# yondonfu/ai-rtc-agent

Hardware: NVIDIA H100
Metric: frames/sec at 512x512 SD-Turbo img2img (1-step, stream-batch 1) (higher is better)
Workload: dtype f16

## Files before the change

ai-rtc-agent_b200/csrc/engine.cu:

```cuda
#include <cuda_fp16.h>
#include <cuda_runtime.h>
#include <math.h>
#include <stddef.h>
#include <stdio.h>
#include <stdlib.h>
#include <string.h>

#include <algorithm>
#include <atomic>
#include <chrono>
#include <functional>
#include <thread>
#include <map>
#include <memory>
#include <string>
#include <vector>

#include "../../include/b200sd.h"
#include "attention.cuh"
#include "elementwise.cuh"
#include "igemm.cuh"
#include "tconv.cuh"

using namespace b2;

namespace b2 {
void igemm_record(const IgemmDesc& g, const IgemmPlan* plan, b2sd_igemm_desc* d, b2sd_igemm_plan_info* info);
}

#define CUDA_OK(expr)                                                                       \
    do {                                                                                    \
        cudaError_t e__ = (expr);                                                           \
        if (e__ != cudaSuccess) {                                                           \
            b2_set_error("%s failed: %s (%s:%d)", #expr, cudaGetErrorString(e__), __FILE__, __LINE__); \
            return -1;                                                                      \
        }                                                                                   \
    } while (0)
#define TRY(expr)            \
    do {                     \
        if ((expr) != 0) return -1; \
    } while (0)

namespace {

struct Act {
    __half* p = nullptr;
    int n = 0, h = 0, w = 0, c = 0, ld = 0;
    long elems() const { return (long)n * h * w * ld; }
};

struct Raw {
    __half* p = nullptr;
    bool pack_only = false;
    bool derived = false;
    std::vector<int64_t> shape;
    std::vector<float> host;
    long numel() const {
        long v = 1;
        for (auto s : shape) v *= s;
        return v;
    }
};

class Arena {
  public:
    explicit Arena(size_t slab) : slab_(slab) {}
    ~Arena() { release(); }
    void set_order(cudaStream_t order, cudaMemPool_t pool) { order_ = order; pool_ = pool; }
    void* alloc(size_t bytes) {
        bytes = (bytes + 1023) & ~size_t(1023);
        if (cur_ < 0 || off_ + bytes > sizes_[cur_]) {
            int next = cur_ + 1;
            while (next < (int)slabs_.size() && sizes_[next] < bytes) ++next;
            if (next >= (int)slabs_.size()) {
                size_t sz = bytes > slab_ ? bytes : slab_;
                void* p = nullptr;
                cudaError_t e = order_ ? cudaMallocFromPoolAsync(&p, sz, pool_, order_) : cudaMalloc(&p, sz);
                if (e == cudaSuccess && order_) e = cudaStreamSynchronize(order_);
                if (e != cudaSuccess) {
                    b2_set_error("device allocation of %zu bytes failed: %s", sz, cudaGetErrorString(e));
                    return nullptr;
                }
                slabs_.push_back(p);
                sizes_.push_back(sz);
                next = (int)slabs_.size() - 1;
            }
            cur_ = next;
            off_ = 0;
        }
        void* r = static_cast<char*>(slabs_[cur_]) + off_;
        off_ += bytes;
        return r;
    }
    void reset() { cur_ = slabs_.empty() ? -1 : 0; off_ = 0; }
    void release() {
        for (void* p : slabs_) order_ ? cudaFreeAsync(p, order_) : cudaFree(p);
        slabs_.clear();
        sizes_.clear();
        cur_ = -1;
        off_ = 0;
    }

  private:
    size_t slab_;
    cudaStream_t order_ = nullptr;
    cudaMemPool_t pool_ = nullptr;
    std::vector<void*> slabs_;
    std::vector<size_t> sizes_;
    int cur_ = -1;
    size_t off_ = 0;
};

struct Op {
    std::function<int(cudaStream_t)> fn;
    std::string name;
    double flops = 0.0;
    b2sd_launch_record rec{};
    template <class F>
    Op(F f, std::string n = "", double fl = 0.0) : fn(std::move(f)), name(std::move(n)), flops(fl) {}
    template <class F>
    Op(F f, std::string n, const b2sd_launch_record& r) : fn(std::move(f)), name(std::move(n)), rec(r) {}
    int operator()(cudaStream_t s) const { return fn(s); }
};

b2sd_launch_record smallconv_record(const SmallConvArgs& a) {
    b2sd_launch_record r{};
    r.kind = B2SD_LAUNCH_SMALLCONV;
    r.smallconv = b2sd_smallconv_args{a.x, a.wt, a.bias, a.y, a.ldy, a.nb, a.h, a.w_, a.cin, a.cout, a.in_h, a.in_w, a.flags,
                                      a.res, a.ldr, (int64_t)a.res_bstride, a.in_off};
    return r;
}
b2sd_launch_record upsample2x_record(const void* x, void* y, int nb, int h, int w, int c) {
    b2sd_launch_record r{};
    r.kind = B2SD_LAUNCH_UPSAMPLE2X;
    r.upsample2x = b2sd_upsample2x_args{x, y, nb, h, w, c};
    return r;
}
b2sd_launch_record post_u8_record(const void* y, int ldy, void* out, int nb, int h, int w) {
    b2sd_launch_record r{};
    r.kind = B2SD_LAUNCH_POST_U8;
    r.post_u8 = b2sd_post_u8_args{y, ldy, out, nb, h, w};
    return r;
}
b2sd_launch_record small_linear_record(const float* in, int in_ld, const void* w, const float* bias, float* out, int out_ld,
                                       int nb, int n, int k, int silu_in) {
    b2sd_launch_record r{};
    r.kind = B2SD_LAUNCH_SMALL_LINEAR;
    r.small_linear = b2sd_small_linear_args{in, in_ld, w, bias, out, out_ld, nb, n, k, silu_in};
    return r;
}

}

static int igemm_autotile_single(IgemmDesc d, bool allow_swap, IgemmPlan* plan_out);

int igemm_autotile(IgemmDesc d, bool allow_swap, IgemmPlan* plan_out) {
    TRY(igemm_autotile_single(d, allow_swap, plan_out));
    static const char* pair_env = getenv("B2_PAIR");
    static const char* ps_env = getenv("B2_PAIR_SPLITS");
    static const bool pair_single = getenv("B2_PAIR_SINGLE") != nullptr;
    const int pair_mode = pair_env ? atoi(pair_env) : d.pair_auto;
    const int pair_splits = ps_env ? atoi(ps_env) : (d.pair_splits > 0 ? d.pair_splits : 4);
    const IgemmPlan& pl = *plan_out;
    const int m_tiles = pl.p.tiles_w * pl.p.tiles_h * pl.p.tiles_n;
    if (pair_mode <= 0 || pl.p.swap || m_tiles < 2 || (pl.p.BN % 32) != 0 || (d.epi.flags & (IG_SILU | IG_PAD0))) return 0;
    if (pair_mode == 2 && pl.p.total_kb < 20) return 0;
    d.swap = 0; d.BN = pl.p.BN; d.splits = pl.splits > pair_splits ? pair_splits : pl.splits; d.partial = nullptr;
    d.pair = pair_single ? 0 : 1;
    IgemmPlan paired;
    if (igemm_plan(d, &paired)) return 0;
    *plan_out = paired;
    return 0;
}

static int igemm_autotile_single(IgemmDesc d, bool allow_swap, IgemmPlan* plan_out) {
    IgemmPlan& plan = *plan_out;
    const bool geglu = (d.epi.flags & IG_GEGLU) != 0;
    const bool silu = (d.epi.flags & IG_SILU) != 0;
    const bool pad0 = (d.epi.flags & IG_PAD0) != 0;
    const int n_gemm = geglu ? 2 * d.epi.n_valid : d.epi.n_valid;
    static const bool swap_on = getenv("B2_SWAP") != nullptr, swap_off = getenv("B2_NO_SWAP") != nullptr;
    static const bool tuned = getenv("B2_NO_TUNED_TILES") == nullptr;
    static const char* ms_env = getenv("B2_MAX_SPLITS");
    const int max_splits = ms_env ? atoi(ms_env) : (d.max_splits > 0 ? d.max_splits : 8);
    int total_kb = 0;
    for (int sidx = 0; sidx < d.nseg && sidx < IG_MAX_SRC; ++sidx) total_kb += d.ntap[sidx] * (d.src[sidx].C / IG_BK);
    const long rows_all = (long)d.Nb * d.Ho * d.Wo;
    const bool swap_here = allow_swap && !geglu && !pad0 && d.epi.n_valid >= 128 && (d.epi.n_valid & 7) == 0 &&
                           (swap_on || (!swap_off && tuned && rows_all <= 64 && total_kb >= 90));
    if (swap_here) {
        d.swap = 1;
        d.BN = rows_all >= 256 ? 256 : (rows_all >= 128 ? 128 : 64);
        d.splits = 1; d.partial = nullptr;
        TRY(igemm_plan(d, &plan));
        const long ctas = (long)plan.grid.x * plan.grid.y;
        int max_by_k = plan.p.total_kb / 4;
        if (max_by_k < 1) max_by_k = 1;
        if (max_by_k > 8) max_by_k = 8;
        int splits = 1;
        while (splits * 2 <= max_by_k && ctas * splits * 2 <= 192 && splits * 2 <= max_splits) splits *= 2;
        if (splits > 1) {
            d.splits = splits;
            TRY(igemm_plan(d, &plan));
        }
        return 0;
    }
    d.swap = 0;
    auto vt_ok = [&](int bn) { return !d.epi.out2 || d.epi.col2 % bn == 0; };
    if (tuned && !geglu && !silu && !pad0 && n_gemm % 160 == 0 && total_kb >= 40 && vt_ok(160)) {
        d.BN = 160; d.splits = 1; d.partial = nullptr;
        TRY(igemm_plan(d, &plan));
        const int m_tiles = plan.p.tiles_w * plan.p.tiles_h * plan.p.tiles_n;
        const long tiles = (long)m_tiles * (n_gemm / 160);
        int bn = 0, splits = 0;
        if (tiles < 132) {
            if (m_tiles >= 8) { bn = 160; splits = 4; }
            else if (m_tiles >= 2 && n_gemm % 256 == 0 && total_kb >= 180 && vt_ok(256)) { bn = 256; splits = 8; }
        }
        if (bn && splits > max_splits) bn = 0;
        if (bn) {
            d.BN = bn; d.splits = splits;
            TRY(igemm_plan(d, &plan));
            return 0;
        }
    }
    static const int cands[] = {256, 160, 128, 64, 32, 16};
    std::vector<int> valid;
    for (int bn : cands) {
        if (geglu && (bn % 32 != 0 || bn < 64)) continue;
        if (silu && (bn > 128 || bn % 16 || (bn & (bn - 1)))) continue;
        if (pad0 && bn != 64 && bn != 128 && bn != 256) continue;
        if (n_gemm % bn == 0 && vt_ok(bn)) valid.push_back(bn);
    }
    if (valid.empty()) {
        int bn = 16;
        while (bn < n_gemm && bn < 128) bn <<= 1;
        valid.push_back(bn);
    }
    for (int bn : valid) {
        if (bn < 64 && n_gemm >= 64) break;
        d.BN = bn; d.splits = 1; d.partial = nullptr;
        TRY(igemm_plan(d, &plan));
        if (plan.p.acc_bufs == 2 || (long)plan.grid.x * plan.grid.y >= b2_device_sms()) return 0;
    }
    int bn = valid.back();
    for (int v : valid) if (v >= 64) bn = v;
    d.BN = bn; d.splits = 1; d.partial = nullptr;
    TRY(igemm_plan(d, &plan));
    const long ctas = (long)plan.grid.x * plan.grid.y;
    int splits = ctas >= 96 ? 1 : (int)((IG_SMS + ctas - 1) / ctas);
    if (tuned && ctas >= 64 && total_kb <= 12) splits = 1;
    const int max_by_k = plan.p.total_kb / 4 > 0 ? plan.p.total_kb / 4 : 1;
    if (splits > max_by_k) splits = max_by_k;
    if (splits > 8) splits = 8;
    while (splits > max_splits && splits > 1) splits >>= 1;
    if (geglu) splits = 1;
    if (splits > 1) {
        d.splits = splits;
        TRY(igemm_plan(d, &plan));
    }
    return 0;
}

struct WeightStore {
    std::shared_ptr<WeightStore> parent;
    struct OrderStream {
        cudaStream_t s = nullptr;
        cudaMemPool_t pool = nullptr;
        ~OrderStream() {
            if (s) cudaStreamDestroy(s);
            if (pool) cudaMemPoolDestroy(pool);
        }
    } order;
    const uint64_t id = next_id();
    uint64_t family = id;
    struct Copy { __half* dst; const __half* src; size_t bytes; };
    std::vector<Copy> pending;
    static uint64_t next_id() {
        static std::atomic<uint64_t> n{1};
        return n++;
    }

    std::map<std::string, Raw> raw;
    Arena weights{256u << 20};
    Arena raw_only{256u << 20};
    bool raw_released = false;
    bool imported = false;
    std::map<std::string, __half*> packed;
    std::map<std::string, float*> fvec;
    std::map<std::string, size_t> packed_bytes, fvec_bytes;
    std::shared_ptr<struct CondPool> cond_pool;

    struct Rebuild {
        std::vector<std::string> keys;
        std::function<int(cudaStream_t)> fn;
    };
    std::map<std::string, Rebuild> rebuild;
    std::map<std::string, const __half*> src_override;
    const __half* src(const std::string& key) const {
        auto o = src_override.find(key);
        if (o != src_override.end()) return o->second;
        auto it = raw.find(key);
        return it == raw.end() ? nullptr : it->second.p;
    }
    bool live = false;
    bool live_ready = false;
    Arena base_arena{256u << 20};
    std::map<std::string, __half*> base;
    std::vector<std::string> fused;
    void* scratch = nullptr;
    size_t scratch_cap = 0;
    ~WeightStore() {
        if (scratch) order.s ? cudaFreeAsync(scratch, order.s) : cudaFree(scratch);
    }
};

enum { COND_PROMPT = 0, COND_TIME = 1 };
static const uint64_t COND_GLOBAL = 0, COND_UNKNOWN = ~0ull;

struct CondPool {
    cudaMemPool_t pool = nullptr;
    cudaStream_t reaper = nullptr;
    ~CondPool() {
// ... 39 lines not shown
    std::map<std::string, Raw>& raw;
    Arena& weights;
    Arena& raw_only;
    bool& raw_released;
    bool& imported;
    std::map<std::string, __half*>& packed;
    std::map<std::string, float*>& fvec;
    std::map<std::string, size_t>& packed_bytes;
    std::map<std::string, size_t>& fvec_bytes;
    Arena state{16u << 20};
    Arena prog{512u << 20};
    explicit b2sd_engine(std::shared_ptr<WeightStore> s)
        : ws(std::move(s)), raw(ws->raw), weights(ws->weights), raw_only(ws->raw_only), raw_released(ws->raw_released),
          imported(ws->imported), packed(ws->packed), fvec(ws->fvec), packed_bytes(ws->packed_bytes), fvec_bytes(ws->fvec_bytes) {}

    Act x_in;
    __half* noise = nullptr;
    float* coef = nullptr;
    float* tsteps = nullptr;
    __half* ctx = nullptr;
    float* temb_sin = nullptr;
    float* temb_h = nullptr;
    float* temb = nullptr;
    float* cn_temb_h = nullptr;
    float* cn_temb = nullptr;
    float* gn_ws = nullptr;
    int* tile_counters = nullptr;
    float coef_host[4][64]{};

    __half* ctx_global = nullptr;
    float* tsteps_global = nullptr;

    struct CondBlock {
        char* p = nullptr;
        char* global = nullptr;
        size_t cap = 0, used = 0;
        uint64_t held = 0;
        void* take(size_t bytes) {
            bytes = (bytes + 1023) & ~size_t(1023);
            if (used + bytes > cap) {
                b2_set_error("conditioning block of %zu bytes exhausted", cap);
                return nullptr;
            }
            void* r = p + used;
            used += bytes;
            return r;
        }
    } cond[2];
    int64_t cond_binds = 0;

    unsigned long long* ln_stats = nullptr;
    size_t ln_stats_cap = 0, ln_stats_used = 0;
    std::vector<Op> prog_frame, prog_prompt, prog_time;
    std::map<std::string, Act> taps;
    SmallConvArgs head{};
    SmallConvArgs cn_head{};
    SmallConvArgs hed_head{};
    Act image;
    bool built = false;
    int concurrency = 1;
    int launches = 0;
    std::string cur;
    bool allow_swap = false;
    size_t idx_enc_end = 0, idx_unet_end = 0;
    enum { GRAPH_WHOLE = 0, GRAPH_STAGE = 1, NUM_GRAPHS = 4 };
    cudaGraphExec_t graph_exec[NUM_GRAPHS] = {};
    void drop_graphs() {
        for (auto& g : graph_exec)
            if (g) { cudaGraphExecDestroy(g); g = nullptr; }
    }

    ~b2sd_engine() { drop_graphs(); }

    const Raw* get(const std::string& key) {
        auto it = raw.find(key);
        if (it == raw.end()) {
            b2_set_error("missing weight '%s'", key.c_str());
            return nullptr;
        }
        return &it->second;
    }
    bool has(const std::string& key) const { return raw.count(key) != 0; }

    float* vec(const std::vector<std::string>& keys, const std::vector<int>* perm = nullptr, int pad_to = 0) {
        std::string ck = "v:";
        for (auto& k : keys) ck += k + "+";
        if (perm) ck += "perm";
        auto it = fvec.find(ck);
        if (it != fvec.end()) return it->second;
        std::vector<float> host;
        for (auto& k : keys) {
            const Raw* r = get(k);
            if (!r) return nullptr;
            if (host.empty()) host.assign(r->host.begin(), r->host.end());
            else
                for (size_t i = 0; i < host.size() && i < r->host.size(); ++i) host[i] += r->host[i];
        }
        if (perm) {
            std::vector<float> t(perm->size());
            for (size_t i = 0; i < perm->size(); ++i) t[i] = (*perm)[i] >= 0 ? host[(*perm)[i]] : 0.f;
            host.swap(t);
        }
        if ((int)host.size() < pad_to) host.resize(pad_to, 0.f);
        float* d = static_cast<float*>(weights.alloc(host.size() * sizeof(float)));
        if (!d) return nullptr;
        if (cudaMemcpy(d, host.data(), host.size() * sizeof(float), cudaMemcpyHostToDevice) != cudaSuccess) return nullptr;
        fvec[ck] = d;
        fvec_bytes[ck] = host.size() * sizeof(float);
        return d;
    }

    const Raw* pack_source(const std::string& key) {
        const Raw* r = get(key);
        if (r && !r->p) {
            b2_set_error("parameter '%s' was released after the first prepare and is not in the packed cache", key.c_str());
            return nullptr;
        }
        return r;
    }
    int record_rebuild(const std::string& name, std::vector<std::string> keys, std::function<int(cudaStream_t)> fn, cudaStream_t s) {
        WeightStore::Rebuild& rb = ws->rebuild[name];
        rb.keys = std::move(keys);
        rb.fn = std::move(fn);
        return rb.fn(s);
    }

    const float* small_w(const std::string& key, cudaStream_t s) {
        auto it = fvec.find("sw:" + key);
        if (it != fvec.end()) return it->second;
        const Raw* r = pack_source(key);
        if (!r) return nullptr;
        const int cout = (int)r->shape[0], cin = (int)r->shape[1];
        float* d = static_cast<float*>(weights.alloc((size_t)cin * 9 * cout * sizeof(float)));
        WeightStore* w = ws.get();
        if (!d || record_rebuild("sw:" + key, {key}, [=](cudaStream_t st) { return smallconv_prep_launch(w->src(key), d, cout, cin, st); }, s))
            return nullptr;
        fvec["sw:" + key] = d;
        fvec_bytes["sw:" + key] = (size_t)cin * 9 * cout * sizeof(float);
        return d;
    }

    struct ConvSeg { std::string key; int c0, cn, taps; };
    __half* pack_conv(const std::string& name, const std::vector<ConvSeg>& segs, int rows, int* k_out,
                      cudaStream_t s) {
        int K = 0;
        for (auto& g : segs) K += g.taps * g.cn;
        *k_out = K;
        auto it = packed.find(name);
        if (it != packed.end()) return it->second;
        const int rows_pad = (rows + 15) / 16 * 16;
        __half* dst = static_cast<__half*>(weights.alloc((size_t)rows_pad * K * 2));
        if (!dst) return nullptr;
        std::vector<std::string> keys;
        std::vector<int> cin_total;
        for (auto& g : segs) {
            const Raw* r = pack_source(g.key);
            if (!r) return nullptr;
            keys.push_back(g.key);
            cin_total.push_back((int)r->shape[1]);
        }
        WeightStore* w = ws.get();
        const size_t bytes = (size_t)rows_pad * K * 2;
        if (record_rebuild(name, keys, [=](cudaStream_t st) {
                if (cudaMemsetAsync(dst, 0, bytes, st) != cudaSuccess) return -1;
                int koff = 0;
                for (size_t i = 0; i < segs.size(); ++i) {
                    const ConvSeg& g = segs[i];
                    if (pack_conv_weight_launch(w->src(g.key), dst, K, koff, rows, cin_total[i], g.taps, g.c0, g.cn, st)) return -1;
                    koff += g.taps * g.cn;
                }
                return 0;
            }, s))
            return nullptr;
        packed[name] = dst;
        packed_bytes[name] = bytes;
        return dst;
    }
    std::function<int(cudaStream_t)> gather_fn(const std::vector<std::pair<std::string, std::vector<int>>>& parts, int K,
                                               __half* dst, size_t bytes, cudaStream_t s) {
        std::vector<std::pair<std::string, const int*>> dparts;
        std::vector<int> counts;
        for (auto& p : parts) {
            if (!pack_source(p.first)) return nullptr;
            int* dperm = static_cast<int*>(weights.alloc(p.second.size() * sizeof(int)));
            if (!dperm) return nullptr;
            cudaMemcpyAsync(dperm, p.second.data(), p.second.size() * sizeof(int), cudaMemcpyHostToDevice, s);
            cudaStreamSynchronize(s);
            dparts.emplace_back(p.first, dperm);
            counts.push_back((int)p.second.size());
        }
        WeightStore* w = ws.get();
        return [=](cudaStream_t st) {
            if (cudaMemsetAsync(dst, 0, bytes, st) != cudaSuccess) return -1;
            size_t r0 = 0;
            for (size_t i = 0; i < dparts.size(); ++i) {
                if (gather_rows_launch(w->src(dparts[i].first), K, dparts[i].second, dst + r0 * K, K, counts[i], K, st)) return -1;
                r0 += counts[i];
            }
            return 0;
        };
    }
    static std::vector<std::string> part_keys(const std::vector<std::pair<std::string, std::vector<int>>>& parts) {
        std::vector<std::string> k;
        for (auto& p : parts) k.push_back(p.first);
        return k;
    }
    __half* pack_rows(const std::string& name, const std::vector<std::pair<std::string, std::vector<int>>>& parts,
                      int K, cudaStream_t s) {
        auto it = packed.find(name);
        if (it != packed.end()) return it->second;
        size_t rows = 0;
        for (auto& p : parts) rows += p.second.size();
        const size_t rows_pad = (rows + 15) / 16 * 16;
        __half* dst = static_cast<__half*>(weights.alloc(rows_pad * K * 2));
        if (!dst) return nullptr;
        auto gather = gather_fn(parts, K, dst, rows_pad * K * 2, s);
        if (!gather || record_rebuild(name, part_keys(parts), gather, s)) return nullptr;
        packed[name] = dst;
        packed_bytes[name] = rows_pad * K * 2;
        return dst;
    }

    struct LnFold { __half* w = nullptr; const float* colsum = nullptr; const float* bias = nullptr; };
    int fold_ln(const std::string& name, const std::vector<std::pair<std::string, std::vector<int>>>& parts, int K,
                const std::string& ln_prefix, const float* bias_vec, LnFold* out, cudaStream_t s) {
        size_t rows = 0;
        for (auto& p : parts) rows += p.second.size();
        const size_t rows_pad = (rows + 15) / 16 * 16;
        const bool done = packed.count(name) && fvec.count(name + ":cs") && fvec.count(name + ":b");
        if (!done) {
            __half* w = static_cast<__half*>(weights.alloc(rows_pad * K * 2));
            if (!w) return -1;
            auto gather = gather_fn(parts, K, w, rows_pad * K * 2, s);
            const float* gamma = vec({ln_prefix + ".weight"});
            const float* beta = vec({ln_prefix + ".bias"});
            float* cs = static_cast<float*>(weights.alloc(rows_pad * sizeof(float)));
            float* bb = static_cast<float*>(weights.alloc(rows_pad * sizeof(float)));
            if (!gather || !gamma || !beta || !cs || !bb) return -1;
            TRY(record_rebuild(name, part_keys(parts), [=](cudaStream_t st) {
                TRY(gather(st));
                if (cudaMemsetAsync(bb, 0, rows_pad * sizeof(float), st) != cudaSuccess) return -1;
                TRY(row_dot_launch(w, (long)rows, K, beta, bias_vec, bb, st));
                TRY(scale_cols_launch(w, (long)rows_pad, K, gamma, st));
                return row_sum_launch(w, (long)rows_pad, K, cs, st);
            }, s));
            packed[name] = w; packed_bytes[name] = rows_pad * K * 2;
            fvec[name + ":cs"] = cs; fvec_bytes[name + ":cs"] = rows_pad * sizeof(float);
            fvec[name + ":b"] = bb; fvec_bytes[name + ":b"] = rows_pad * sizeof(float);
        }
        out->w = packed[name];
        out->colsum = fvec[name + ":cs"];
        out->bias = fvec[name + ":b"];
        return 0;
    }
    unsigned long long* alloc_rowstat(long rows) {
        if (ln_stats_used + 2 * (size_t)rows > ln_stats_cap) {
            b2_set_error("LayerNorm statistics slab exhausted");
            return nullptr;
        }
        unsigned long long* p = ln_stats + ln_stats_used;
        ln_stats_used += 2 * (size_t)rows;
        return p;
    }

    Act new_act(int n, int h, int w, int c, int ld = 0) {
        Act a;
        a.n = n; a.h = h; a.w = w; a.c = c; a.ld = ld ? ld : c;
        a.p = static_cast<__half*>(prog.alloc((size_t)a.elems() * 2));
        return a;
    }
    static ActView view(const Act& a) { return ActView{a.p, a.n, a.h, a.w, a.c, a.ld}; }
    static ActView tokens(const Act& a) { return ActView{a.p, 1, 1, a.n * a.h * a.w, a.c, a.ld}; }

    void push_igemm(std::vector<Op>& dst, const IgemmDesc& d, const IgemmPlan& plan, const std::string& label, double flops) {
        if (&dst == &prog_frame) launches += 1;
        dst.push_back(Op([plan](cudaStream_t s) { return igemm_launch(plan, s); }, label, flops));
        dst.back().rec.kind = B2SD_LAUNCH_IGEMM;
        igemm_record(d, &plan, &dst.back().rec.igemm, &dst.back().rec.plan);
    }

    void push_attn(const AttnPlan& plan, const std::string& label) {
        const AttnDesc& a = plan.d;
        launches += 1;
        prog_frame.push_back(Op([plan](cudaStream_t st) { return attn_launch(plan, st); }, label,
                                4.0 * a.nb * a.heads * (double)a.sq * a.skv * a.d_real));
        b2sd_launch_record& r = prog_frame.back().rec;
        r.kind = B2SD_LAUNCH_ATTN;
        r.attn = b2sd_attn_desc{a.q, a.ldq, a.k, a.ldk, (int64_t)a.k_bstride, (int64_t)a.k_rows, a.vt, a.ldvt, (int64_t)a.vt_bstride,
                                (int64_t)a.vt_cols, a.out, a.ldo, a.nb, a.heads, a.sq, a.skv, a.d_real, a.dp};
    }

    int add_igemm(std::vector<Op>& dst, IgemmDesc d) {
        const bool geglu = (d.epi.flags & IG_GEGLU) != 0;
        const int n_gemm = geglu ? 2 * d.epi.n_valid : d.epi.n_valid;
        const bool extras = d.epi.rowstat_out || d.epi.colsum || d.epi.out2;
        if (concurrency > 1 && d.max_splits == 0) d.max_splits = 4;
        if (concurrency >= 4 && d.pair_auto == 0) { d.pair_auto = 1; d.pair_splits = 1; }
        IgemmPlan plan;
        TRY(igemm_autotile(d, allow_swap && !extras, &plan));
        if (d.epi.out2 && d.epi.col2 % plan.p.BN != 0) {
            b2_set_error("fused q/k/v projection: N tile %d does not divide the V offset %d", plan.p.BN, d.epi.col2);
            return -1;
        }
        char label[256];
        snprintf(label, sizeof(label), "igemm %s rows=%ld n=%d kb=%d bn=%d splits=%d grid=%u,%u,%u %s", cur.c_str(),
                 plan.rows_total, d.epi.n_valid, plan.p.total_kb, plan.p.BN, plan.splits, plan.grid.x, plan.grid.y,
                 plan.grid.z, plan.p.swap ? "swapped" : (plan.pair ? "pairs" : "taps"));
        push_igemm(dst, d, plan, label, 2.0 * (double)plan.rows_total * n_gemm * plan.p.total_kb * IG_BK);
        return 0;
    }

    int add_groupnorm(const Act& xa, const Act* xb, const std::string& prefix, const Act& y, float eps, int silu) {
        GroupNormArgs a{};
        a.xa = xa.p; a.ca = xa.c; a.lda = xa.ld;
        if (xb) { a.xb = xb->p; a.cb = xb->c; a.ldb = xb->ld; }
        a.gamma = vec({prefix + ".weight"});
        a.beta = vec({prefix + ".bias"});
        if (!a.gamma || !a.beta) return -1;
        a.y = y.p; a.ldy = y.ld;
        a.nb = xa.n; a.hw = xa.h * xa.w; a.groups = cfg.norm_groups; a.eps = eps; a.silu = silu;
        a.partial = gn_ws;
        a.counters = tile_counters;
        launches += 1;
        prog_frame.push_back(Op([a](cudaStream_t s) { return groupnorm_launch(a, s); }, "groupnorm " + prefix));
        b2sd_launch_record& r = prog_frame.back().rec;
        r.kind = B2SD_LAUNCH_GROUPNORM;
        r.groupnorm = b2sd_groupnorm_args{a.xa, a.ca, a.lda, a.xb, a.cb, a.ldb, a.gamma, a.beta, a.y, a.ldy, a.nb, a.hw, a.groups,
                                          a.eps, a.silu};
        return 0;
    }

    int add_layernorm(const Act& x, const std::string& prefix, const Act& y) {
        const float* g = vec({prefix + ".weight"});
        const float* b = vec({prefix + ".bias"});
        if (!g || !b) return -1;
        const long rows = (long)x.n * x.h * x.w;
        const __half* xp = x.p; __half* yp = y.p;
        const int ldx = x.ld, ldy = y.ld, c = x.c;
        ++launches;
        prog_frame.push_back(Op([=](cudaStream_t s) { return layernorm_launch(xp, ldx, g, b, yp, ldy, rows, c, 1e-5f, s); }, "layernorm " + prefix));
        b2sd_launch_record& r = prog_frame.back().rec;
        r.kind = B2SD_LAUNCH_LAYERNORM;
        r.layernorm = b2sd_layernorm_args{xp, ldx, g, b, yp, ldy, (int64_t)rows, c, 1e-5f};
        return 0;
    }

    int add_conv(std::vector<Op>& dst, const Act& x, const std::string& wkey, const std::string& bkey, int taps,
                 int stride, const Act& y, int flags, const Act* res, cudaStream_t s, float acc_scale = 1.f,
                 float res_scale = 1.f) {
        const Raw* w = get(wkey);
        if (!w) return -1;
        cur = wkey;
        const int cout = (int)w->shape[0];
        int K = 0;
        __half* wp = pack_conv(wkey, {{wkey, 0, x.c, taps}}, cout, &K, s);
        if (!wp) return -1;
        IgemmDesc d{};
        d.nseg = 1; d.src[0] = view(x); d.ntap[0] = taps;
        d.w = wp; d.w_rows = (cout + 15) / 16 * 16; d.w_ld = K;
        d.stride = stride;
        d.Nb = y.n; d.Ho = y.h; d.Wo = y.w;
        d.epi.out = y.p; d.epi.ldc = y.ld;
        if (!bkey.empty()) {
            d.epi.colbias = vec({bkey}, nullptr, 16);
            if (!d.epi.colbias) return -1;
        }
        d.epi.colbias_bstride = 0;
        if (res) { d.epi.res = res->p; d.epi.ldr = res->ld; }
        d.epi.acc_scale = acc_scale; d.epi.res_scale = res_scale;
        d.epi.flags = flags;
        d.epi.n_valid = cout;
        static const bool no_tconv = getenv("B2_NO_TCONV") != nullptr;
        static const char* tc_min = getenv("B2_TCONV_MIN_TILES");
        const long tiles = (long)y.n * ((y.h + TC_TH - 1) / TC_TH) * ((y.w + TC_TW - 1) / TC_TW);
        if (!no_tconv && stride == 1 && tconv_eligible(d) && tiles >= (tc_min ? atoi(tc_min) : 2 * IG_SMS)) {
            TconvPlan tp;
            TRY(tconv_plan(d, &tp));
            char label[256];
            snprintf(label, sizeof(label), "tconv %s rows=%ld tiles=%d grid=%u nbuf=%d", wkey.c_str(), tp.rows_total, tp.p.num_tiles,
                     tp.grid.x, tp.p.nbuf);
            if (&dst == &prog_frame) launches += 1;
            dst.push_back(Op([tp](cudaStream_t st) { return tconv_launch(tp, st); }, label, 2.0 * (double)tp.rows_total * cout * K));
            dst.back().rec.kind = B2SD_LAUNCH_TCONV;
            igemm_record(d, nullptr, &dst.back().rec.igemm, &dst.back().rec.plan);
            return 0;
        }
        return add_igemm(dst, d);
    }

    struct LinExtra {
        unsigned long long* rowstat_out = nullptr;
        const unsigned long long* rowstat_in = nullptr;
        const float* colsum = nullptr;
        int ln_c = 0;
        __half* out2 = nullptr;
        int ld2 = 0, col2 = 0;
    };
    int add_linear(std::vector<Op>& dst, const ActView& x, const __half* w, int n, int k, const float* bias,
                   __half* out, int ldc, const __half* res, int ldr, int flags = 0, int n_valid = -1,
                   const LinExtra* ex = nullptr) {
        IgemmDesc d{};
        if (ex) {
            d.epi.rowstat_out = ex->rowstat_out;
            d.epi.rowstat_in = ex->rowstat_in;
            d.epi.colsum = ex->colsum;
            d.epi.ln_inv_c = ex->ln_c ? 1.f / (float)ex->ln_c : 0.f;
            d.epi.ln_eps = 1e-5f;
            d.epi.out2 = ex->out2; d.epi.ld2 = ex->ld2; d.epi.col2 = ex->col2;
        }
        d.nseg = 1; d.src[0] = x; d.ntap[0] = 1;
        d.w = w; d.w_rows = n; d.w_ld = k;
        d.stride = 1;
        d.Nb = 1; d.Ho = 1; d.Wo = x.W;
        d.epi.out = out; d.epi.ldc = ldc;
        d.epi.colbias = bias; d.epi.colbias_bstride = 0;
        d.epi.res = res; d.epi.ldr = ldr;
        d.epi.acc_scale = 1.f; d.epi.res_scale = 1.f;
        d.epi.flags = flags;
        d.epi.n_valid = n_valid >= 0 ? n_valid : n;
        return add_igemm(dst, d);
    }

    int build_resnet(const std::string& p, const Act& xa, const Act* xb, int cout, const float* emb, Act* out, cudaStream_t s,
                     float eps = 1e-5f);
    int build_vae_attention(const std::string& p, const Act& x, Act* out, cudaStream_t s);
    int build_kl_encoder(Act* out, std::string* latent_conv, cudaStream_t s);
    int build_kl_decoder(const Act& x0, cudaStream_t s);
    std::vector<float> host_copy(const std::string& key);
    int derive(const std::string& name, const std::vector<int64_t>& shape, const std::vector<float>& v);
    const float* const_vec(const std::string& name, const std::vector<float>& v);
    int build_cond_embedding(Act* out, cudaStream_t s);
    int build_hed(const uint8_t** control, cudaStream_t s);
    int build_controlnet(const Act& cond, std::vector<Act>& skips, Act* mid, cudaStream_t s);
    int build_transformer(const std::string& p, const Act& x, int heads, Act* out, cudaStream_t s);
    int build_taesd_block(const std::string& p, const Act& x, Act* out, cudaStream_t s);
    int build_program(cudaStream_t s);
    int run(std::vector<Op>& ops, cudaStream_t s, size_t a = 0, size_t b = SIZE_MAX) {
        static const bool dbg = getenv("B200SD_DEBUG_SYNC") != nullptr;
        static const char* skip = getenv("B200SD_SKIP");
        static const char* skip_name = getenv("B200SD_SKIP_NAME");
        for (size_t idx = a; idx < b && idx < ops.size(); ++idx) {
            Op& op = ops[idx];
            if (skip) {
                const std::string kind = op.name.substr(0, op.name.find(' '));
                if (!kind.empty() && std::string(skip).find(kind) != std::string::npos) continue;
            }
            if (skip_name && op.name.find(skip_name) != std::string::npos) continue;
            TRY(op(s));
            if (dbg) {
                cudaError_t e = cudaStreamSynchronize(s);
                if (e != cudaSuccess) {
                    b2_set_error("op %zu '%s' failed: %s", idx, op.name.c_str(), cudaGetErrorString(e));
                    fprintf(stderr, "b2sd: op %zu '%s' failed: %s\n", idx, op.name.c_str(), cudaGetErrorString(e));
                    return -1;
                }
            }
        }
        return 0;
    }
};

int b2sd_engine::build_resnet(const std::string& p, const Act& xa, const Act* xb, int cout, const float* emb, Act* out,
                              cudaStream_t s, float eps) {
    cur = p;
    allow_swap = true;
    const int cin = xa.c + (xb ? xb->c : 0);
    const int B = xa.n;
    Act n1 = new_act(B, xa.h, xa.w, cin);
    TRY(add_groupnorm(xa, xb, p + "norm1", n1, eps, 1));
    Act h1 = new_act(B, xa.h, xa.w, cout);
    {
        int K = 0;
        __half* wp = pack_conv(p + "conv1.weight", {{p + "conv1.weight", 0, cin, 9}}, cout, &K, s);
        if (!wp) return -1;
        const float* colbias = nullptr;
        if (emb) {
            float* cb = static_cast<float*>(cond[COND_TIME].take((size_t)B * cout * sizeof(float)));
            const float* bsum = vec({p + "conv1.bias", p + "time_emb_proj.bias"});
            const Raw* wt = get(p + "time_emb_proj.weight");
            if (!cb || !bsum || !wt) return -1;
            const int tdim = (int)wt->shape[1];
            const __half* wtp = wt->p;
            prog_time.push_back(Op([=](cudaStream_t st) { return small_linear_launch(emb, tdim, wtp, bsum, cb, cout, B, cout, tdim, 1, st); }, "temb " + p,
                                   small_linear_record(emb, tdim, wtp, bsum, cb, cout, B, cout, tdim, 1)));
            colbias = cb;
        } else {
            colbias = vec({p + "conv1.bias"}, nullptr, 16);
            if (!colbias) return -1;
        }
        IgemmDesc d{};
        d.nseg = 1; d.src[0] = view(n1); d.ntap[0] = 9;
        d.w = wp; d.w_rows = cout; d.w_ld = K; d.stride = 1;
        d.Nb = B; d.Ho = xa.h; d.Wo = xa.w;
        d.epi.out = h1.p; d.epi.ldc = h1.ld;
        d.epi.colbias = colbias; d.epi.colbias_bstride = emb ? cout : 0;
        d.epi.acc_scale = 1.f; d.epi.res_scale = 1.f; d.epi.n_valid = cout;
        TRY(add_igemm(prog_frame, d));
    }
    Act n2 = new_act(B, xa.h, xa.w, cout);
    TRY(add_groupnorm(h1, nullptr, p + "norm2", n2, eps, 1));
    *out = new_act(B, xa.h, xa.w, cout);
    IgemmDesc d{};
    d.stride = 1; d.Nb = B; d.Ho = xa.h; d.Wo = xa.w;
    d.epi.out = out->p; d.epi.ldc = out->ld;
    d.epi.acc_scale = 1.f; d.epi.res_scale = 1.f; d.epi.n_valid = cout;
    d.src[0] = view(n2); d.ntap[0] = 9;
    int K = 0;
    if (has(p + "conv_shortcut.weight")) {
        std::vector<ConvSeg> segs = {{p + "conv2.weight", 0, cout, 9}, {p + "conv_shortcut.weight", 0, xa.c, 1}};
        d.nseg = 2; d.src[1] = view(xa); d.ntap[1] = 1;
        if (xb) {
            segs.push_back({p + "conv_shortcut.weight", xa.c, xb->c, 1});
            d.nseg = 3; d.src[2] = view(*xb); d.ntap[2] = 1;
        }
        __half* wp = pack_conv(p + "conv2+shortcut", segs, cout, &K, s);
        if (!wp) return -1;
        d.w = wp; d.w_rows = cout; d.w_ld = K;
        d.epi.colbias = vec({p + "conv2.bias", p + "conv_shortcut.bias"});
    } else {
        if (xb) {
            b2_set_error("resnet %s: concat input without conv_shortcut", p.c_str());
            return -1;
        }
        __half* wp = pack_conv(p + "conv2.weight", {{p + "conv2.weight", 0, cout, 9}}, cout, &K, s);
        if (!wp) return -1;
        d.nseg = 1;
        d.w = wp; d.w_rows = cout; d.w_ld = K;
        d.epi.colbias = vec({p + "conv2.bias"});
        d.epi.res = xa.p; d.epi.ldr = xa.ld;
    }
    if (!d.epi.colbias) return -1;
    return add_igemm(prog_frame, d);
}

int b2sd_engine::build_transformer(const std::string& p, const Act& x, int heads, Act* out, cudaStream_t s) {
    cur = p;
    allow_swap = true;
    const int B = x.n, C = x.c, HW = x.h * x.w;
    const long M = (long)B * HW;
    const int d_real = C / heads;
    const int dp = d_real <= 64 ? 64 : (d_real <= 128 ? 128 : 192);
    const int Cp = heads * dp;
    const int D = cfg.cross_attention_dim, L = cfg.ctx_tokens;
    const std::string t = p + "transformer_blocks.0.";
    auto head_perm = [&](int base) {
        std::vector<int> pm(Cp);
        for (int hh = 0; hh < heads; ++hh)
            for (int i = 0; i < dp; ++i) pm[hh * dp + i] = i < d_real ? base + hh * d_real + i : -1;
        return pm;
    };
    Act n = new_act(B, x.h, x.w, C);
    TRY(add_groupnorm(x, nullptr, p + "norm", n, 1e-6f, 0));
    const int HWp = (HW + 7) / 8 * 8;
    const bool one_gemm = (HW % 8 == 0) || B == 1;
    static const bool no_fold = getenv("B2_NO_LNFOLD") != nullptr;
    static const char* fold_rows_env = getenv("B2_LNFOLD_MAX_ROWS");
    const long fold_max_rows = fold_rows_env ? atol(fold_rows_env) : (1l << 40);
    const bool fold = !no_fold && one_gemm && (long)B * (cfg.height / 8) * (cfg.width / 8) <= fold_max_rows;
    const int inner = 4 * C;
    std::vector<int> gperm;
    {
        const int half = 64;
        for (int tI = 0; tI < inner / half; ++tI) {
            for (int i = 0; i < half; ++i) gperm.push_back(tI * half + i);
            for (int i = 0; i < half; ++i) gperm.push_back(inner + tI * half + i);
        }
    }
    const float* bff1 = vec({t + "ff.net.0.proj.bias"}, &gperm);
    if (!bff1) return -1;
    const Raw* wpi = get(p + "proj_in.weight");
    if (!wpi) return -1;
    Act hs = new_act(B, x.h, x.w, C);
    unsigned long long *st1 = nullptr, *st2 = nullptr, *st3 = nullptr;
    if (fold) {
        st1 = alloc_rowstat(M); st2 = alloc_rowstat(M); st3 = alloc_rowstat(M);
        if (!st1 || !st2 || !st3) return -1;
    }
    {
        LinExtra ex; ex.rowstat_out = st1;
        TRY(add_linear(prog_frame, tokens(n), wpi->p, C, C, vec({p + "proj_in.bias"}), hs.p, C, nullptr, 0, 0, -1, &ex));
    }
    Act qk = new_act(1, 1, (int)M, 2 * Cp);
    const long vt_ld = one_gemm ? (M + 7) / 8 * 8 : (long)B * HWp;
    const long vt_bstride = one_gemm ? HW : HWp;
    __half* vt = static_cast<__half*>(prog.alloc((size_t)Cp * vt_ld * 2));
    if (!vt) return -1;
    cudaMemsetAsync(vt, 0, (size_t)Cp * vt_ld * 2, s);
    if (fold) {
        LnFold f;
        TRY(fold_ln(t + "attn1.qkv+ln", {{t + "attn1.to_q.weight", head_perm(0)}, {t + "attn1.to_k.weight", head_perm(0)},
                                         {t + "attn1.to_v.weight", head_perm(0)}}, C, t + "norm1", nullptr, &f, s));
        LinExtra ex; ex.rowstat_in = st1; ex.colsum = f.colsum; ex.ln_c = C; ex.out2 = vt; ex.ld2 = (int)vt_ld; ex.col2 = 2 * Cp;
        TRY(add_linear(prog_frame, tokens(hs), f.w, 3 * Cp, C, f.bias, qk.p, 2 * Cp, nullptr, 0, 0, -1, &ex));
    } else {
        Act ln = new_act(B, x.h, x.w, C);
        TRY(add_layernorm(hs, t + "norm1", ln));
        __half* wqk = pack_rows(t + "attn1.qk", {{t + "attn1.to_q.weight", head_perm(0)}, {t + "attn1.to_k.weight", head_perm(0)}}, C, s);
        __half* wv = pack_rows(t + "attn1.v", {{t + "attn1.to_v.weight", head_perm(0)}}, C, s);
        if (!wqk || !wv) return -1;
        TRY(add_linear(prog_frame, tokens(ln), wqk, 2 * Cp, C, nullptr, qk.p, 2 * Cp, nullptr, 0));
        allow_swap = false;
        for (int bi = 0; bi < (one_gemm ? 1 : B); ++bi) {
            ActView wv_view{wv, 1, 1, Cp, C, C};
            IgemmDesc d{};
            d.nseg = 1; d.src[0] = wv_view; d.ntap[0] = 1;
            d.w = one_gemm ? ln.p : ln.p + (long)bi * HW * ln.ld;
            d.w_rows = one_gemm ? (int)M : HW; d.w_ld = C; d.stride = 1;
            d.Nb = 1; d.Ho = 1; d.Wo = Cp;
            d.epi.out = one_gemm ? vt : vt + (long)bi * HWp;
            d.epi.ldc = (int)vt_ld; d.epi.acc_scale = 1.f; d.epi.res_scale = 1.f;
            d.epi.n_valid = one_gemm ? (int)M : HW;
// ... 2119 lines not shown
```

Baseline: 200.1.

## Add halo-tile implicit-GEMM kernel for stride-1 3x3 convolutions

Adds a new conv kernel for stride-1 3x3 convolutions. It loads one haloed spatial tile (8x16 plus border) per channel block via TMA, then runs all nine taps as WGMMA descriptors offset within that shared-memory tile, so activations are not re-fetched per tap. Weights are multicast across a CTA pair over a deep staged pipeline. Eligible igemm ops with a plain epilogue and no split-K or swap are routed to it. The risks are lower occupancy from the large shared-memory footprint, less split-K parallelism on small layers, and possible issues with descriptor offsets into the swizzled halo buffer.

Result: no change. 201.2 (median of 6 runs) (+0.6%).

```diff
diff --git a/ai-rtc-agent_b200/csrc/engine.cu b/ai-rtc-agent_b200/csrc/engine.cu
--- a/ai-rtc-agent_b200/csrc/engine.cu
+++ b/ai-rtc-agent_b200/csrc/engine.cu
@@ -19,6 +19,7 @@
 #include "../../include/b200sd.h"
 #include "attention.cuh"
 #include "elementwise.cuh"
+#include "hconv.cuh"
 #include "igemm.cuh"
 #include "tconv.cuh"
 
@@ -664,11 +665,23 @@
             b2_set_error("fused q/k/v projection: N tile %d does not divide the V offset %d", plan.p.BN, d.epi.col2);
             return -1;
         }
+        const double flops = 2.0 * (double)plan.rows_total * n_gemm * plan.p.total_kb * IG_BK;
         char label[256];
+        if (hconv_routable(d, plan)) {
+            HconvPlan hp;
+            TRY(hconv_plan(d, plan, &hp));
+            snprintf(label, sizeof(label), "igemm %s rows=%ld n=%d kb=%d bn=%d splits=1 grid=%u,%u,1 halo", cur.c_str(),
+                     plan.rows_total, d.epi.n_valid, plan.p.total_kb, plan.p.BN, hp.grid.x, hp.grid.y);
+            if (&dst == &prog_frame) launches += 1;
+            dst.push_back(Op([hp](cudaStream_t s) { return hconv_launch(hp, s); }, label, flops));
+            dst.back().rec.kind = B2SD_LAUNCH_IGEMM;
+            igemm_record(d, &plan, &dst.back().rec.igemm, &dst.back().rec.plan);
+            return 0;
+        }
         snprintf(label, sizeof(label), "igemm %s rows=%ld n=%d kb=%d bn=%d splits=%d grid=%u,%u,%u %s", cur.c_str(),
                  plan.rows_total, d.epi.n_valid, plan.p.total_kb, plan.p.BN, plan.splits, plan.grid.x, plan.grid.y,
                  plan.grid.z, plan.p.swap ? "swapped" : (plan.pair ? "pairs" : "taps"));
-        push_igemm(dst, d, plan, label, 2.0 * (double)plan.rows_total * n_gemm * plan.p.total_kb * IG_BK);
+        push_igemm(dst, d, plan, label, flops);
         return 0;
     }
 
diff --git a/ai-rtc-agent_b200/csrc/hconv.cu b/ai-rtc-agent_b200/csrc/hconv.cu
--- /dev/null
+++ b/ai-rtc-agent_b200/csrc/hconv.cu
@@ -0,0 +1,255 @@
+#include "hconv.cuh"
+
+#include "epilogue.cuh"
+#include "launch.cuh"
+#include "ptx.cuh"
+
+namespace b2 {
+
+template <int BN>
+__global__ void __launch_bounds__(IG_THREADS, 1) hconv_kernel(const __grid_constant__ HconvParams p) {
+    extern __shared__ uint8_t smem_raw[];
+    uint8_t* smem = reinterpret_cast<uint8_t*>((reinterpret_cast<uintptr_t>(smem_raw) + 1023) & ~static_cast<uintptr_t>(1023));
+    const int warp = threadIdx.x >> 5;
+    const int lane = threadIdx.x & 31;
+    constexpr uint32_t W_BYTES = (uint32_t)BN * IG_BK * 2;
+    uint8_t* sW = smem;
+    uint8_t* sA = smem + (size_t)p.wstages * W_BYTES;
+    uint64_t* w_full = reinterpret_cast<uint64_t*>(sA + 2 * HC_ABUF);
+    uint64_t* w_empty = w_full + HC_MAX_W;
+    uint64_t* a_full = w_empty + HC_MAX_W;
+    uint64_t* a_empty = a_full + 2;
+    const int cr = (int)(blockIdx.x & 1);
+    const int ntile = blockIdx.y;
+
+    if (threadIdx.x == IG_CONS) {
+        for (int s = 0; s < p.nseg; ++s) tma_prefetch_desc(&p.tmA[s]);
+        tma_prefetch_desc(&p.tmB);
+        for (int s = 0; s < p.wstages; ++s) {
+            mbar_init(&w_full[s], 1);
+            mbar_init(&w_empty[s], 2 * (IG_CONS / 32));
+        }
+        for (int s = 0; s < 2; ++s) {
+            mbar_init(&a_full[s], 1);
+            mbar_init(&a_empty[s], IG_CONS / 32);
+        }
+        fence_mbar_init();
+    }
+    cluster_arrive_relaxed();
+    cluster_wait();
+    __syncthreads();
+
+    pdl_launch_dependents();
+    pdl_wait();
+
+    if (warp == IG_CONS / 32) {
+        if (lane == 0) {
+            const uint16_t pair_mask = (uint16_t)(3u << (cluster_ctarank() & ~1u));
+            int ws = 0, as = 0;
+            uint32_t wph = 0, aph = 0;
+            for (int mt = blockIdx.x; mt - cr < p.num_mtiles; mt += gridDim.x) {
+                const int w0 = (mt % p.tiles_w) * HC_TW, h0 = ((mt / p.tiles_w) % p.tiles_h) * HC_TH;
+                const int n0 = mt / (p.tiles_w * p.tiles_h);
+                for (int seg = 0; seg < p.nseg; ++seg) {
+                    const int ntap = p.seg_ntap[seg];
+                    const int halo = ntap == 9 ? 1 : 0;
+                    for (int cb = 0; cb < p.seg_cblocks[seg]; ++cb) {
+                        mbar_wait(&a_empty[as], aph ^ 1);
+                        mbar_expect_tx(&a_full[as], halo ? HC_HALO_BYTES : HC_PLAIN_BYTES);
+                        tma_load_4d(sA + (size_t)as * HC_ABUF, &p.tmA[seg], &a_full[as], cb * IG_BK, w0 - halo, h0 - halo, n0);
+                        if (++as == 2) {
+                            as = 0;
+                            aph ^= 1;
+                        }
+                        for (int tap = 0; tap < ntap; ++tap) {
+                            mbar_wait(&w_empty[ws], wph ^ 1);
+                            mbar_expect_tx(&w_full[ws], W_BYTES);
+                            tma_load_2d_mc(sW + (size_t)ws * W_BYTES + cr * (BN / 2) * 128, &p.tmB, &w_full[ws],
+                                           (p.seg_kb0[seg] + tap * p.seg_cblocks[seg] + cb) * IG_BK, ntile * BN + cr * (BN / 2),
+                                           pair_mask);
+                            if (++ws == p.wstages) {
+                                ws = 0;
+                                wph ^= 1;
+                            }
+                        }
+                    }
+                }
+            }
+        }
+    } else {
+        const int wg = warp >> 2;
+        const int r0 = wg * 64 + (warp & 3) * 16 + (lane >> 2);
+        const uint32_t peer_empty = dsmem_map(smem_u32(w_empty), cluster_ctarank() ^ 1u);
+        const uint32_t sw_base = smem_u32(sW), sa_base = smem_u32(sA);
+        auto release_w = [&](int s) {
+            if (lane == 0) {
+                mbar_arrive(&w_empty[s]);
+                mbar_arrive_remote(peer_empty + (uint32_t)s * 8u);
+            }
+        };
+        auto release_a = [&](int s) {
+            if (lane == 0) mbar_arrive(&a_empty[s]);
+        };
+        int ws = 0, as = 0;
+        uint32_t wph = 0, aph = 0;
+        for (int mt = blockIdx.x; mt - cr < p.num_mtiles; mt += gridDim.x) {
+            float acc[BN / 2];
+#pragma unroll
+            for (int i = 0; i < BN / 2; ++i) acc[i] = 0.f;
+            int prev_w = -1, prev_a = -1;
+            for (int seg = 0; seg < p.nseg; ++seg) {
+                const int ntap = p.seg_ntap[seg];
+                for (int cb = 0; cb < p.seg_cblocks[seg]; ++cb) {
+                    mbar_wait(&a_full[as], aph);
+                    const uint32_t a0 = sa_base + (uint32_t)as * HC_ABUF;
+                    for (int tap = 0; tap < ntap; ++tap) {
+                        mbar_wait(&w_full[ws], wph);
+                        const uint64_t da = ntap == 9
+                            ? make_kmajor_sw128_desc(a0 + (uint32_t)(((8 * wg + tap / 3) * (HC_TW + 2) + tap % 3) * 128), (HC_TW + 2) * 128)
+                            : make_kmajor_sw128_desc(a0 + (uint32_t)wg * (64 * 128));
+                        const uint64_t db = make_kmajor_sw128_desc(sw_base + (uint32_t)ws * W_BYTES);
+                        wgmma_fence_regs(acc);
+                        wgmma_fence();
+#pragma unroll
+                        for (int k = 0; k < 4; ++k) Wgmma<BN>::ss(acc, da + 2 * k, db + 2 * k, 1u);
+                        wgmma_commit();
+                        wgmma_wait<1>();
+                        wgmma_fence_regs(acc);
+                        if (prev_w >= 0) release_w(prev_w);
+                        prev_w = ws;
+                        if (tap == 0 && prev_a >= 0) {
+                            release_a(prev_a);
+                            prev_a = -1;
+                        }
+                        if (++ws == p.wstages) {
+                            ws = 0;
+                            wph ^= 1;
+                        }
+                    }
+                    prev_a = as;
+                    if (++as == 2) {
+                        as = 0;
+                        aph ^= 1;
+                    }
+                }
+            }
+            wgmma_wait<0>();
+            wgmma_fence_regs(acc);
+            if (prev_w >= 0) release_w(prev_w);
+            if (prev_a >= 0) release_a(prev_a);
+
+            const int w0 = (mt % p.tiles_w) * HC_TW, h0 = ((mt / p.tiles_w) % p.tiles_h) * HC_TH;
+            const int n0 = mt / (p.tiles_w * p.tiles_h);
+            EpiRow rw[2];
+#pragma unroll
+            for (int h = 0; h < 2; ++h) {
+                const int r = r0 + 8 * h;
+                const int hh = h0 + (r >> 3), ww = w0 + (r & 7);
+                rw[h].ok = n0 < p.Nb && hh < p.Ho && ww < p.Wo;
+                rw[h].orow = ((long)n0 * p.Ho + hh) * p.Wo + ww;
+                rw[h].b = n0;
+                rw[h].mu = 0.f;
+                rw[h].rstd = 1.f;
+            }
+            epi_frag<BN>(p.epi, acc, rw, ntile, false, lane);
+        }
+    }
+    cluster_arrive_relaxed();
+    cluster_wait();
+}
+
+using HconvFn = void (*)(HconvParams);
+static HconvFn hconv_fn(int bn) {
+    switch (bn) {
+        case 64: return hconv_kernel<64>;
+        case 128: return hconv_kernel<128>;
+        case 160: return hconv_kernel<160>;
+        default: return nullptr;
+    }
+}
+
+int igemm_encode_act_map(CUtensorMap* m, const ActView& a, int box_c, int box_w, int box_h, int box_n, int estride);
+int igemm_encode_w_map(CUtensorMap* m, const __half* w, int rows, int ld, int box_rows);
+
+static long hconv_mtiles(const IgemmDesc& d) {
+    return (long)((d.Wo + HC_TW - 1) / HC_TW) * ((d.Ho + HC_TH - 1) / HC_TH) * d.Nb;
+}
+
+bool hconv_routable(const IgemmDesc& d, const IgemmPlan& pl) {
+    const IgEpilogue& e = d.epi;
+    if (!pl.pair || pl.splits != 1 || pl.p.swap || !hconv_fn(pl.p.BN) || d.stride > 1 || d.nseg < 1 || d.nseg > IG_MAX_SRC) return false;
+    if ((e.flags & (IG_GEGLU | IG_SPLITK | IG_SILU | IG_PAD0)) || e.colsum || e.rowstat_in || e.rowstat_out || e.out2) return false;
+    bool any3 = false;
+    for (int s = 0; s < d.nseg; ++s) {
+        const ActView& a = d.src[s];
+        if (d.ntap[s] == 9) any3 = true;
+        if (a.N != d.Nb || a.H != d.Ho || a.W != d.Wo || a.C % IG_BK) return false;
+    }
+    return any3 && hconv_mtiles(d) <= (long)pl.p.tiles_w * pl.p.tiles_h * pl.p.tiles_n;
+}
+
+int hconv_plan(const IgemmDesc& d, const IgemmPlan& pl, HconvPlan* plan) {
+    *plan = HconvPlan{};
+    if (!hconv_routable(d, pl)) {
+        b2_set_error("hconv: needs a CTA-pair plan without split-K (N tile 64 / 128 / 160) of stride-1 segments over the output's "
+                     "extent with a plain epilogue");
+        return -1;
+    }
+    HconvParams& p = plan->p;
+    const int BN = pl.p.BN;
+    p.nseg = d.nseg;
+    int kb = 0;
+    for (int s = 0; s < d.nseg; ++s) {
+        const bool halo = d.ntap[s] == 9;
+        p.seg_ntap[s] = d.ntap[s];
+        p.seg_cblocks[s] = d.src[s].C / IG_BK;
+        p.seg_kb0[s] = kb;
+        kb += d.ntap[s] * p.seg_cblocks[s];
+        if (igemm_encode_act_map(&p.tmA[s], d.src[s], IG_BK, HC_TW + 2 * halo, HC_TH + 2 * halo, 1, 1)) return -1;
+    }
+    if (igemm_encode_w_map(&p.tmB, d.w, d.w_rows, d.w_ld, BN / 2)) return -1;
+    p.tiles_w = (d.Wo + HC_TW - 1) / HC_TW;
+    p.tiles_h = (d.Ho + HC_TH - 1) / HC_TH;
+    p.num_mtiles = p.tiles_w * p.tiles_h * d.Nb;
+    p.Wo = d.Wo; p.Ho = d.Ho; p.Nb = d.Nb;
+    p.BN = BN;
+    p.epi = d.epi;
+    const size_t w_bytes = (size_t)BN * IG_BK * 2;
+    const size_t fixed = 2 * (size_t)HC_ABUF + 1024  + 512 ;
+    int st = (int)((227 * 1024 - fixed) / w_bytes);
+    p.wstages = st > HC_MAX_W ? HC_MAX_W : st;
+    plan->smem = fixed + (size_t)p.wstages * w_bytes;
+    const int n_tiles = (int)pl.grid.y;
+    int gx = (p.num_mtiles + 1) & ~1;
+    const int wave = (b2_device_sms() / n_tiles) & ~1;
+    if (gx > wave && wave >= 2) gx = wave;
+    plan->grid = dim3(gx, n_tiles, 1);
+    return 0;
+}
+
+int hconv_launch(const HconvPlan& plan, cudaStream_t stream) {
+    static bool attr_set = false;
+    HconvFn fn = hconv_fn(plan.p.BN);
+    if (!fn) {
+        b2_set_error("hconv launch: no kernel for BN %d", plan.p.BN);
+        return -1;
+    }
+    if (!attr_set) {
+        for (int bn : {64, 128, 160}) {
+            cudaError_t e = cudaFuncSetAttribute(hconv_fn(bn), cudaFuncAttributeMaxDynamicSharedMemorySize, 227 * 1024);
+            if (e != cudaSuccess) {
+                b2_set_error("cudaFuncSetAttribute(hconv BN %d): %s", bn, cudaGetErrorString(e));
+                return -1;
+            }
+        }
+        attr_set = true;
+    }
+    cudaError_t e = launch_kc(fn, plan.grid, dim3(IG_THREADS), plan.smem, stream, 2, 1, plan.p);
+    if (e != cudaSuccess) {
+        b2_set_error("hconv launch: %s", cudaGetErrorString(e));
+        return -1;
+    }
+    return 0;
+}
+
+}
diff --git a/ai-rtc-agent_b200/csrc/hconv.cuh b/ai-rtc-agent_b200/csrc/hconv.cuh
--- /dev/null
+++ b/ai-rtc-agent_b200/csrc/hconv.cuh
@@ -0,0 +1,35 @@
+#pragma once
+#include "igemm.cuh"
+
+namespace b2 {
+
+constexpr int HC_TW = 8, HC_TH = 16;
+constexpr int HC_MAX_W = 12;
+constexpr uint32_t HC_HALO_BYTES = (HC_TW + 2) * (HC_TH + 2) * IG_BK * 2;
+constexpr uint32_t HC_PLAIN_BYTES = HC_TW * HC_TH * IG_BK * 2;
+constexpr uint32_t HC_ABUF = (HC_HALO_BYTES + 1023u) & ~1023u;
+
+struct HconvParams {
+    CUtensorMap tmA[IG_MAX_SRC];
+    CUtensorMap tmB;
+    int seg_ntap[IG_MAX_SRC];
+    int seg_cblocks[IG_MAX_SRC];
+    int seg_kb0[IG_MAX_SRC];
+    int nseg;
+    int tiles_w, tiles_h, num_mtiles;
+    int Wo, Ho, Nb;
+    int BN, wstages;
+    IgEpilogue epi;
+};
+
+struct HconvPlan {
+    HconvParams p;
+    dim3 grid;
+    size_t smem;
+};
+
+bool hconv_routable(const IgemmDesc& d, const IgemmPlan& pl);
+int hconv_plan(const IgemmDesc& d, const IgemmPlan& pl, HconvPlan* plan);
+int hconv_launch(const HconvPlan& plan, cudaStream_t stream);
+
+}
```
